# ZhangXiaze/DeepPointMap

Hardware: AMD Instinct MI355X
Metric: LiDAR frames/s (encode+match+register), 65 536 pts/frame (higher is better)
Workload: dtype f32 (attention scores K Q^T and P V, Linear / Conv1d (+ LayerNorm) layers with K <= 2048 as exact three-way bf16 splits: 6 bf16 products per fp32 product, fp32 accumulate -- fp32 accuracy, bf16 matrix pipe; all else fp32); 1 GPU; synthetic 64x65536-pt scans per GPU: Encoder.forward + consecutive-frame registration_forward (256x256) + information matrix per frame; points_per_frame=65536, parallelism=frame-sharded x1, one RCCL gather of descriptors+edges per step, weights=procedural (deeppointmap_amd/weights.py), allocator_reserve_gib=16, geometry_waits_for_caller_stream=True

## Files before the change

deeppointmap_amd/_lib.py:

```python
from __future__ import annotations

import ctypes
import os

import torch
from ctypes import c_char_p, c_double, c_int, c_longlong, c_size_t, c_uint, c_void_p

_HERE = os.path.dirname(os.path.abspath(__file__))
LIB_PATH = os.environ.get("DPM_LIB") or os.path.join(_HERE, "libdpm_hip.so")
VERSION_EXPERIMENT = 0x40000000

P, I, D, LL = c_void_p, c_int, c_double, c_longlong

SIGNATURES = {
    "dpm_version": (I, []),
    "dpm_error_string": (c_char_p, [I]),
    "dpm_prepare_points": (I, [P, P, I, I, I, P, P, P]),
    "dpm_to_channel_first": (I, [P, I, I, I, P, P]),
    "dpm_to_channel_first_ld": (I, [P, I, I, I, P, I, P]),
    "dpm_emit_descriptors": (I, [P, P, P, I, I, I, D, P, P, P, P, P]),
    "dpm_nested_levels": (I, [P, P, I, I, I, P, P, P, P, P]),
    "dpm_gather_frames": (I, [P, LL, I, I, I, P, I, P, P]),
    "dpm_fps_workspace_bytes": (c_size_t, [I, I, I]),
    "dpm_fps": (I, [P, P, I, I, I, P, P, P, P, P]),
    "dpm_fps_ex": (I, [P, P, I, I, I, P, P, P, P, I, P]),
    "dpm_fps_start": (I, [P, P, P, I, I, I, P, P, P, P, P]),
    "dpm_knn_workspace_bytes": (c_size_t, [I, I]),
    "dpm_knn_hybrid": (I, [P, P, P, I, I, I, I, D, P, P, P]),
    "dpm_knn_hybrid_reuse": (I, [P, P, P, I, I, I, I, D, P, P, P, P, P]),
    "dpm_knn_build_grid": (I, [P, P, I, I, D, P, P]),
    "dpm_knn_hybrid_prebuilt": (I, [P, P, P, I, I, I, I, D, P, P, P]),
    "dpm_ball_query": (I, [P, P, P, I, I, I, I, D, P, P]),
    "dpm_voxel_sampler_bounds": (I, [P, P, I, I, I, D, D, P, P]),
    "dpm_voxel_sampler_workspace_bytes": (c_size_t, [I, I, LL]),
    "dpm_voxel_sampler_select": (I, [P, P, I, I, I, D, D, P, LL, I, P, I, P, P, P]),
    "dpm_posegraph_optimize": (I, [P, I, P, P, P, P, I, I, P, P, P]),
    "dpm_host_topk_replay": (I, [P, I, I, I, P]),
    "dpm_host_sort_replay": (I, [P, I, I, P]),
    "dpm_group_mlp_max": (I, [P, P, P, P, P, P, P, P, I, I, I, I, I, I, D, P, P]),
    "dpm_group_mlp_max_generic": (I, [P, P, P, P, P, P, P, P, I, I, I, I, I, I, D, P, P]),
    "dpm_group_mlp_max_from_xyz": (I, [P, P, P, P, P, P, P, P, P, I, I, I, I, I, I, D, P, P]),
    "dpm_group_gather_ln_max": (I, [P, P, P, P, P, I, P, P, I, I, I, I, I, D, P, P]),
    "dpm_group_gather_ln_max_folded": (I, [P, P, P, P, I, P, P, I, I, I, I, I, D, P, P]),
    "dpm_group_affine_ln_max": (I, [P, P, P, P, P, P, I, P, P, I, I, I, I, I, D, P, P]),
    "dpm_group_gather_ln_max_centred": (I, [P, P, P, P, I, P, P, I, I, I, I, I, D, P, P]),
    "dpm_group_affine_ln_max_centred": (I, [P, P, P, P, P, P, I, P, P, I, I, I, I, I, D, P, P]),
    "dpm_linear": (I, [P, I, P, I, P, P, I, P, I, I, I, I, I, P]),
    "dpm_linear_batched": (I, [P, I, LL, P, I, LL, P, P, I, LL, P, I, LL, I, I, I, I, I, P]),
    "dpm_split_bf16x3": (I, [P, LL, P, P]),
    "dpm_linear_bf16x3": (I, [P, I, P, I, LL, P, P, I, P, I, I, I, I, I, P]),
    "dpm_linear_bf16x3_rank3": (I, [P, I, P, I, LL, P, P, I, P, I, I, I, I, I, P, P, I, D, P]),
    "dpm_linear_layernorm_bf16x3": (I, [P, I, P, I, LL, P, P, P, P, P, P, I, I, I, I, I, P]),
    "dpm_pwconv_pair_bf16x3": (I, [P, I, P, LL, P, P, P, P, LL, P, P, P, P, P, I, I, I, P]),
    "dpm_decoder_tail_bf16x3": (I, [P, P, P, P, I, I, P, LL, P, P, P, P, LL, P, P, LL, P, P, P, P]),
    "dpm_layernorm": (I, [P, I, P, P, P, P, P, I, I, I, I, P]),
    "dpm_linear_layernorm": (I, [P, I, P, I, P, P, P, P, P, P, I, I, I, I, I, P]),
    "dpm_three_interp_cat": (I, [P, P, P, P, P, I, I, I, I, I, P, P]),
    "dpm_posemb": (I, [P, I, P, I, I, I, P, P]),
    "dpm_attention": (I, [P, I, LL, P, I, LL, P, I, LL, P, I, LL, I, I, I, I, I, P]),
    "dpm_attention_shifted": (I, [P, I, LL, P, I, LL, P, I, LL, P, I, LL, I, I, I, I, I, I, P]),
    "dpm_attention_masked": (I, [P, I, LL, P, I, LL, P, I, LL, P, I, LL, I, I, I, I, I, I, P, P]),
    "dpm_attention_indexed": (I, [P, I, LL, P, I, LL, P, I, LL, P, I, LL, I, I, I, I, I, I, P, P]),
    "dpm_attention_split_workspace_bytes": (c_size_t, [I, I, I, I, I]),
    "dpm_attention_planes_bytes": (c_size_t, [I, I, I]),
    "dpm_attention_planes": (I, [P, I, LL, P, P, I, LL, I, I, I, I, I, P, P]),
    "dpm_linear_bf16x3_kvplanes": (I, [P, I, P, I, LL, P, P, I, I, I, I, I, I, I, P, P]),
    "dpm_attention_split": (I, [P, I, LL, P, I, LL, P, I, LL, P, I, LL, I, I, I, I, I, I, I, P, P]),
    "dpm_l2_normalize": (I, [P, I, I, P, P]),
    "dpm_match_workspace_bytes": (c_size_t, [I, I, I, I]),
    "dpm_match_topk": (I, [P, P, I, I, I, I, D, I, P, P, P, P]),
    "dpm_pairing_workspace_bytes": (c_size_t, [I, I, I]),
    "dpm_dual_softmax_topk": (I, [P, I, I, I, D, I, P, P, P, P]),
    "dpm_gather_pairs": (I, [P, P, P, I, I, I, I, I, P, P, P, P]),
    "dpm_mean_rows": (I, [P, I, I, I, P, I, P]),
    "dpm_kabsch_workspace_bytes": (c_size_t, [I, I]),
    "dpm_corr_kabsch": (I, [P, P, I, LL, P, I, LL, P, P, P, I, I, D, I, D, P, P, P, I, P]),
    "dpm_preprocess_workspace_bytes": (c_size_t, [LL]),
    "dpm_preprocess_scan": (I, [P, I, I, D, D, D, D, LL, P, P, I, P, P, P]),
    "dpm_knn_self_workspace_bytes": (c_size_t, [I]),
    "dpm_knn_self": (I, [P, I, I, D, P, P, P, P, P]),
    "dpm_point_normals": (I, [P, I, D, P, P, P]),
    "dpm_lowpass_similarity": (I, [P, P, I, I, I, P, P]),
    "dpm_stat_filter": (I, [P, I, D, I, D, P, P, P, P, P, P]),
    "dpm_filter_dc_workspace_bytes": (c_size_t, [I, I]),
    "dpm_outlier_filter_dc": (I, [P, P, P, I, I, D, D, D, P, P, P, P, P]),
    "dpm_lowpass_filter_dc": (I, [P, P, P, I, D, I, D, I, D, D, P, P, P, P, P]),
    "dpm_augment_workspace_bytes": (c_size_t, [I, LL]),
    "dpm_ground_filter": (I, [P, P, P, I, I, I, D, D, I, P, P, P, P, P]),
    "dpm_voxel_select": (I, [P, P, P, I, D, I, LL, P, P, P, P, P]),
    "dpm_mask_select": (I, [P, P, P, I, I, D, D, P, D, P, I, P, P, P, P, P]),
    "dpm_points_affine": (I, [P, P, I, I, P, P, P]),
    "dpm_points_deskew": (I, [P, P, P, I, I, P, I, I, P, D, P]),
    "dpm_gather_points": (I, [P, P, P, I, P, I, I, P, P, P, P]),
    "dpm_pack_frames": (I, [P, P, P, I, I, P, P, P, P]),
    "dpm_ingest_frames": (I, [P, P, LL, I, I, I, P, P, P, P, P]),
    "dpm_map_tile": (I, [P, P, P, P, I, I, I, P, P]),
    "dpm_infomat_workspace_bytes": (c_size_t, [I, I, I]),
    "dpm_information_matrix": (I, [P, I, P, I, P, D, P, P, P]),
    "dpm_information_matrix_batched": (I, [P, I, P, P, I, P, I, D, P, I, P, P]),
    "dpm_infomat_build_grids": (I, [P, I, P, I, D, P, P]),
    "dpm_infomat_search_grids": (I, [P, I, P, P, I, P, I, D, P, I, P, P]),
    "dpm_icp_workspace_bytes": (c_size_t, [I, I]),
    "dpm_icp_refine_batched": (I, [P, I, I, P, P, P, P, I, P, I, P, P, I, D, D, P, P, P, P, P, P, P, P, P]),
    "dpm_voxel_map_workspace_bytes": (c_size_t, [LL]),
    "dpm_voxel_map_init": (I, [LL, P, P]),
    "dpm_voxel_map_bounds": (I, [P, P, P, I, LL, P, P]),
# ... 121 lines not shown
```

deeppointmap_amd/csrc/gemm_b3.hip:

```cpp
#include "dpm_common.h"
#include <type_traits>

namespace {

using bf16x8 = __attribute__((ext_vector_type(8))) __bf16;
using f32x4 = __attribute__((ext_vector_type(4))) float;
using u32x4 = __attribute__((ext_vector_type(4))) unsigned;
using u32x2 = __attribute__((ext_vector_type(2))) unsigned;

__device__ __forceinline__ float b3_act(float v, int act) {
    if (act == DPM_ACT_RELU) return fmaxf(v, 0.f);
    if (act == DPM_ACT_SIGMOID) return 1.f / (1.f + __expf(-v));
    return v;
}

__global__ __launch_bounds__(256) void split_bf16x3_kernel(const float *__restrict__ W, long long n, uint16_t *__restrict__ planes) {
    const long long i = (long long)blockIdx.x * 256 + threadIdx.x;
    if (i >= n) return;
    unsigned h, m, l;
    split3(W[i], h, m, l);
    planes[i] = (uint16_t)(h >> 16), planes[n + i] = (uint16_t)(m >> 16), planes[2 * n + i] = (uint16_t)(l >> 16);
}

#ifndef DPM_B3_WIDE
// ... 689 lines not shown
        f32x4 y[2] = {f32x4{0.f, 0.f, 0.f, 0.f}, f32x4{0.f, 0.f, 0.f, 0.f}};
#pragma unroll
        for (int s4 = 0; s4 < PW_H / 32; ++s4) {
            unsigned hh[8], mm[8], ll[8];
#pragma unroll
            for (int e = 0; e < 8; ++e) split3(h[2 * s4 + (e >> 2)][e & 3], hh[e], mm[e], ll[e]);
            bf16x8 hb[3];
            hb[0] = __builtin_bit_cast(bf16x8, u32x4{pack2(hh[0], hh[1]), pack2(hh[2], hh[3]), pack2(hh[4], hh[5]), pack2(hh[6], hh[7])});
            hb[1] = __builtin_bit_cast(bf16x8, u32x4{pack2(mm[0], mm[1]), pack2(mm[2], mm[3]), pack2(mm[4], mm[5]), pack2(mm[6], mm[7])});
            hb[2] = __builtin_bit_cast(bf16x8, u32x4{pack2(ll[0], ll[1]), pack2(ll[2], ll[3]), pack2(ll[4], ll[5]), pack2(ll[6], ll[7])});
            bf16x8 a[2][3];
#pragma unroll
            for (int jj = 0; jj < 2; ++jj)
#pragma unroll
                for (int pl = 0; pl < 3; ++pl)
                    a[jj][pl] = *reinterpret_cast<const bf16x8 *>(&W2s[pl][s4][jj * 16 + fr][b3_col(fr, 8 * g)]);
#define DPM_PW2(PWQ, PXQ)                                                                             \
    _Pragma("unroll") for (int jj = 0; jj < 2; ++jj)                                                  \
        y[jj] = __builtin_amdgcn_mfma_f32_16x16x32_bf16(a[jj][PWQ], hb[PXQ], y[jj], 0, 0, 0)
            DPM_PW2(1, 1);
            DPM_PW2(2, 0);
            DPM_PW2(0, 2);
            DPM_PW2(1, 0);
            DPM_PW2(0, 1);
            DPM_PW2(0, 0);
#undef DPM_PW2
        }
        float s2 = 0.f;
#pragma unroll
        for (int jj = 0; jj < 2; ++jj) {
            const f32x4 bv = *reinterpret_cast<const f32x4 *>(&vec2[0][16 * jj + 4 * g]);
#pragma unroll
            for (int q = 0; q < 4; ++q) y[jj][q] += bv[q], s2 += y[jj][q];
        }
        const float mu2 = pw_rows4_sum(s2) * (1.f / PW_C);
        float q2 = 0.f;
#pragma unroll
        for (int jj = 0; jj < 2; ++jj)
#pragma unroll
            for (int q = 0; q < 4; ++q) y[jj][q] -= mu2, q2 = fmaf(y[jj][q], y[jj][q], q2);
        const float rs2 = rsqrtf(pw_rows4_sum(q2) * (1.f / PW_C) + 1e-5f);
        if (row0 + fr < R) {
#pragma unroll
            for (int jj = 0; jj < 2; ++jj) {
                const f32x4 gv = *reinterpret_cast<const f32x4 *>(&vec2[1][16 * jj + 4 * g]);
                const f32x4 ev = *reinterpret_cast<const f32x4 *>(&vec2[2][16 * jj + 4 * g]);
                const f32x4 pv = jj ? p1 : p0;
                f32x4 o;
#pragma unroll
                for (int q = 0; q < 4; ++q) o[q] = fmaxf(fmaf(y[jj][q] * rs2, gv[q], ev[q]) + pv[q], 0.f);
                *reinterpret_cast<f32x4 *>(out + (size_t)row * PW_C + 16 * jj + 4 * g) = o;
            }
        }
    }
}

}

extern "C" int dpm_split_bf16x3(const float *W, long long n, void *planes, dpm_stream_t stream) {
    DPM_CHECK_ARG(W && planes && n >= 1);
    hipLaunchKernelGGL(split_bf16x3_kernel, dim3(dpm_cdiv(n, 256)), dim3(256), 0, (hipStream_t)stream, W, n, (uint16_t *)planes);
    return dpm_launch_status();
}

extern "C" int dpm_linear_bf16x3_rank3(const float *x, int ldx, const void *w_planes, int ldw, long long plane_stride,
                                       const float *bias, const float *residual, int ldr, float *out, int ldo, int R, int Cin,
                                       int Cout, int act, const float *x3, const float *w3, int ldw3, double scale,
                                       dpm_stream_t stream);

extern "C" int dpm_linear_bf16x3(const float *x, int ldx, const void *w_planes, int ldw, long long plane_stride, const float *bias,
                                 const float *residual, int ldr, float *out, int ldo, int R, int Cin, int Cout, int act,
                                 dpm_stream_t stream) {
    return dpm_linear_bf16x3_rank3(x, ldx, w_planes, ldw, plane_stride, bias, residual, ldr, out, ldo, R, Cin, Cout, act, nullptr,
                                   nullptr, 0, 0.0, stream);
}

extern "C" int dpm_linear_bf16x3_rank3(const float *x, int ldx, const void *w_planes, int ldw, long long plane_stride,
                                       const float *bias, const float *residual, int ldr, float *out, int ldo, int R, int Cin,
                                       int Cout, int act, const float *x3, const float *w3, int ldw3, double scale,
                                       dpm_stream_t stream) {
    DPM_CHECK_ARG((x3 == nullptr) == (w3 == nullptr) && (!x3 || ldw3 >= 3));
    const float r3s = (float)scale;
    DPM_CHECK_ARG(x && w_planes && out && R >= 1 && Cin >= 1 && Cout >= 1 && ldx >= Cin && ldw >= Cin && ldo >= Cout);
    DPM_CHECK_ARG(act >= DPM_ACT_NONE && act <= DPM_ACT_SIGMOID && (!residual || ldr >= Cout) && plane_stride >= (long long)Cout * ldw);
    auto al = [](const void *p) { return ((uintptr_t)p & 15) == 0; };
    if (Cin % B3_KT != 0 || Cout % 4 != 0 || ldw % 8 != 0 || plane_stride % 8 != 0 || ldo % 4 != 0 || !al(w_planes) || !al(out) ||
        !al(bias) || (residual && (!al(residual) || ldr % 4 != 0)))
        return DPM_EUNSUPPORTED;
    const bool xvec = ldx % 4 == 0 && al(x);
    const long long big = (long long)dpm_cdiv(R, 64) * dpm_cdiv(Cout, 64);
#define DPM_B3_LAUNCH(TM, TN, V, PF)                                                                                          \
    hipLaunchKernelGGL((gemm_b3_kernel<TM, TN, V, PF>), dim3(dpm_cdiv(Cout, TN), dpm_cdiv(R, TM)), dim3(256), 0, (hipStream_t)stream, x, ldx, \
                       (const uint16_t *)w_planes, ldw, plane_stride, bias, residual, ldr, out, ldo, R, Cin, Cout, act, x3, w3, ldw3, r3s)
    if (DPM_B3_WIDE && xvec && Cout % 128 == 0 && (long long)dpm_cdiv(R, 64) * (Cout / 128) >= DPM_B3_WIDE) {
        DPM_B3_LAUNCH(64, 128, true, 1);
    } else if (big >= 192 || (R > 1024 && Cout > 32)) {
        const bool small = big <= DPM_B3_DEEP;
        if (xvec && small) DPM_B3_LAUNCH(64, 64, true, 4);
        else if (xvec) DPM_B3_LAUNCH(64, 64, true, 1);
        else if (small) DPM_B3_LAUNCH(64, 64, false, 4);
        else DPM_B3_LAUNCH(64, 64, false, 1);
    } else {
        const bool small = (long long)dpm_cdiv(R, 32) * dpm_cdiv(Cout, 32) <= 2 * DPM_B3_DEEP;
        if (xvec && small) DPM_B3_LAUNCH(32, 32, true, 4);
        else if (xvec) DPM_B3_LAUNCH(32, 32, true, 1);
        else if (small) DPM_B3_LAUNCH(32, 32, false, 4);
// ... 33 lines not shown
    auto al = [](const void *p) { return ((uintptr_t)p & 15) == 0; };
    if (Cin % B3_KT != 0 || ldx % 4 != 0 || ldw % 8 != 0 || plane_stride % 8 != 0 || ldo % 4 != 0 || !al(x) || !al(w_planes) ||
        !al(bias) || !al(pre) || !al(gamma) || !al(beta) || !al(post) || !al(out))
        return DPM_EUNSUPPORTED;
    hipStream_t st = (hipStream_t)stream;
#define DPM_GLN3(BM, BN, WGM, WGN)                                                                                             \
    hipLaunchKernelGGL((gemm_ln_b3_kernel<BM, BN, WGM, WGN>), dim3(dpm_cdiv(R, BM)), dim3(64 * WGM * WGN), 0, st, x, ldx,       \
                       (const uint16_t *)w_planes, ldw, plane_stride, bias, pre, gamma, beta, post, out, ldo, R, Cin, act)
    if (Cout == 256) DPM_GLN3(64, 256, 2, 4);
    else if (Cout == 128) DPM_GLN3(64, 128, 2, 2);
    else if (Cout == 64) DPM_GLN3(64, 64, 2, 2);
    else if (Cout == 32) DPM_GLN3(64, 32, 2, 2);
    else return DPM_EUNSUPPORTED;
#undef DPM_GLN3
    return dpm_launch_status();
}

#ifndef DPM_TAIL_ZREG
#define DPM_TAIL_ZREG 0
#endif
extern "C" int dpm_decoder_tail_bf16x3(const float *a, const float *pre, const float *post, float *out, int R, int C,
                                       const void *wo_planes, long long plane_o, const float *bo, const float *g2, const float *be2,
                                       const void *w0_planes, long long plane_0, const float *b0, const void *w2_planes,
                                       long long plane_2, const float *b2, const float *g3, const float *be3, dpm_stream_t stream) {
    DPM_CHECK_ARG(a && pre && out && wo_planes && w0_planes && w2_planes && g2 && be2 && g3 && be3 && R >= 1 && C >= 1 && a != out);
    const long long cc = (long long)C * C;
    DPM_CHECK_ARG(plane_o >= cc && plane_0 >= cc && plane_2 >= cc);
    auto al = [](const void *p) { return ((uintptr_t)p & 15) == 0; };
    if (C != DT_C || plane_o % 8 != 0 || plane_0 % 8 != 0 || plane_2 % 8 != 0 || !al(a) || !al(pre) || !al(post) || !al(out) ||
        !al(wo_planes) || !al(w0_planes) || !al(w2_planes) || !al(bo) || !al(b0) || !al(b2) || !al(g2) || !al(be2) || !al(g3) || !al(be3))
        return DPM_EUNSUPPORTED;
    const TailArgs A{a, pre, post, out, {(const uint16_t *)wo_planes, (const uint16_t *)w0_planes, (const uint16_t *)w2_planes},
                     {plane_o, plane_0, plane_2}, {bo, b0, b2}, g2, be2, g3, be3, R};
    hipLaunchKernelGGL(decoder_tail_b3_kernel<DPM_TAIL_ZREG != 0>, dim3(dpm_cdiv(R, DT_BM)), dim3(DT_T), 0, (hipStream_t)stream, A);
    return dpm_launch_status();
}

extern "C" int dpm_pwconv_pair_bf16x3(const float *x, int ldx, const void *w1_planes, long long plane1, const float *b1,
                                      const float *g1, const float *be1, const void *w2_planes_kperm, long long plane2,
                                      const float *b2, const float *g2, const float *be2, const float *post, float *out, int R,
                                      int C, int H, dpm_stream_t stream) {
    DPM_CHECK_ARG(x && w1_planes && w2_planes_kperm && g1 && be1 && g2 && be2 && out && R >= 1 && ldx >= C);
    auto al = [](const void *p) { return ((uintptr_t)p & 15) == 0; };
    if (C != PW_C || H != PW_H || ldx % 4 != 0 || plane1 % 8 != 0 || plane2 % 8 != 0 || !al(x) || !al(w1_planes) ||
        !al(w2_planes_kperm) || !al(post) || !al(out))
        return DPM_EUNSUPPORTED;
    const long long tiles = ((long long)R + 15) / 16;
    const int tpw = (int)std::max<long long>(1, (tiles + 4LL * DPM_PW_GRID - 1) / (4LL * DPM_PW_GRID));
    const unsigned grid = (unsigned)((tiles + 4LL * tpw - 1) / (4LL * tpw));
    hipLaunchKernelGGL(pwconv_pair_b3_kernel, dim3(grid), dim3(256), 0, (hipStream_t)stream, x, ldx, (const uint16_t *)w1_planes,
                       plane1, b1, g1, be1, (const uint16_t *)w2_planes_kperm, plane2, b2, g2, be2, post, out, R, tpw);
    return dpm_launch_status();
}
```

deeppointmap_amd/knobs.py:

```python
from __future__ import annotations

import os

FPS_ALGO = None
FUSED_LN = True
GEMM_BF16X3 = True
BF16X3_MAX_K = 2048
GEMM_LN_BF16X3 = True
BF16X3_LN_MIN_K = 128
FUSED_LN_SMALL_ROWS = 0
FOLD_GATHER = True
FOLD_MIN_RADIUS = 0.2
CENTRED_GATHER = True
FUSED_PWCONV = True
FUSED_MATCH = True
KV_PLANES = True
DECODER_TAIL_FUSED = True
DEDUP_FRAMES = True

_ENV = {"DPM_FOLD_MIN_RADIUS": ("FOLD_MIN_RADIUS", float), "DPM_KV_PLANES": ("KV_PLANES", lambda v: v != "0"), "DPM_CENTRED_GATHER": ("CENTRED_GATHER", lambda v: v != "0"), "DPM_FPS_ALGO": ("FPS_ALGO", int), "DPM_NO_FUSED_LN": ("FUSED_LN", lambda v: v != "1"),
        "DPM_DEDUP_FRAMES": ("DEDUP_FRAMES", lambda v: v != "0"), "DPM_DECODER_TAIL": ("DECODER_TAIL_FUSED", lambda v: v != "0"), "DPM_GEMM_BF16X3": ("GEMM_BF16X3", lambda v: v == "1"), "DPM_BF16X3_MAX_K": ("BF16X3_MAX_K", int), "DPM_BF16X3_LN_MIN_K": ("BF16X3_LN_MIN_K", int), "DPM_FUSED_LN_SMALL_ROWS": ("FUSED_LN_SMALL_ROWS", int), "DPM_GEMM_LN_BF16X3": ("GEMM_LN_BF16X3", lambda v: v == "1"),
        "DPM_FUSED_MATCH": ("FUSED_MATCH", lambda v: v != "0"), "DPM_FUSED_PWCONV": ("FUSED_PWCONV", lambda v: v != "0"), "DPM_FOLD_GATHER": ("FOLD_GATHER", lambda v: v != "0")}


def env_knobs() -> dict:
    return {k: v for k, v in sorted(os.environ.items()) if k.startswith("DPM_")}


def apply_env() -> dict:
    g = globals()
    for var, (name, conv) in _ENV.items():
        if var in os.environ:
            g[name] = conv(os.environ[var])
    return env_knobs()
```

deeppointmap_amd/ops.py:

```python
from __future__ import annotations

from typing import Optional, Tuple

import ctypes
import threading
import weakref

import torch

from . import _lib, knobs

ACT_NONE, ACT_RELU, ACT_SIGMOID = 0, 1, 2


def _ptr(t: Optional[torch.Tensor]):
    return None if t is None else t.data_ptr()


def _stream(t: torch.Tensor):
    return torch.cuda.current_stream(t.device).cuda_stream


def _chk(t: torch.Tensor, dtype, name: str):
    if not t.is_cuda:
# ... 470 lines not shown

def linear_layernorm(x: torch.Tensor, W: torch.Tensor, bias: Optional[torch.Tensor], gamma: torch.Tensor, beta: torch.Tensor,
                     act: int = ACT_NONE, pre: Optional[torch.Tensor] = None, post: Optional[torch.Tensor] = None) -> torch.Tensor:
    Cout, Cin = W.shape[0], W.shape[1]
    x2 = x.reshape(-1, x.shape[-1])
    if (knobs.GEMM_BF16X3 and knobs.GEMM_LN_BF16X3 and Cin % 32 == 0 and knobs.BF16X3_LN_MIN_K <= Cin <= knobs.BF16X3_MAX_K and Cout % 4 == 0 and W.numel() == Cout * Cin
            and x.dtype == torch.float32):
        wp = _weight_planes(W)
        if wp is not None and (bias is None or bias.data_ptr() % 16 == 0):
            if (Cout in FUSED_LN_WIDTHS and (x2.shape[0] >= FUSED_LN_MIN_ROWS or x2.shape[0] <= knobs.FUSED_LN_SMALL_ROWS)
                    and x2.is_contiguous() and knobs.FUSED_LN):
                planes, off, n = wp
                out = torch.empty(*x.shape[:-1], Cout, device=x.device, dtype=torch.float32)
                for nm, t in (("pre", pre), ("post", post)):
                    if t is not None:
                        _chk(t, torch.float32, nm)
                        if t.numel() != out.numel():
                            raise ValueError(f"{nm} must have the shape of the output")
                st = _lib.load().dpm_linear_layernorm_bf16x3(_ptr(x2), x2.stride(0), planes.data_ptr() + 2 * off, Cin, n, _ptr(bias),
                                                             _ptr(pre), _ptr(gamma), _ptr(beta), _ptr(post), _ptr(out), Cout,
                                                             x2.shape[0], Cin, Cout, act, _stream(x))
                if st == 0:
                    return out
                if st != -2:
                    _lib.check(st, "dpm_linear_layernorm_bf16x3")
            y = linear_bf16x3(x, W, bias, residual=pre)
            if y is not None:
                return layernorm(y, gamma, beta, act=act, post=post)
    if (Cout in FUSED_LN_WIDTHS and x2.shape[0] >= FUSED_LN_MIN_ROWS and W.is_contiguous() and x2.is_contiguous()
            and x.dtype == torch.float32 and Cin % 4 == 0 and knobs.FUSED_LN):
        _chk(W, torch.float32, "W")
        out = torch.empty(*x.shape[:-1], Cout, device=x.device, dtype=torch.float32)
        for n, t in (("pre", pre), ("post", post)):
            if t is not None:
                _chk(t, torch.float32, n)
                if t.numel() != out.numel():
                    raise ValueError(f"{n} must have the shape of the output")
        st = _lib.load().dpm_linear_layernorm(_ptr(x2), x2.stride(0), _ptr(W), Cin, _ptr(bias), _ptr(pre), _ptr(gamma),
                                              _ptr(beta), _ptr(post), _ptr(out), Cout, x2.shape[0], Cin, Cout, act, _stream(x))
        if st == 0:
            return out
        if st != -2:
            _lib.check(st, "dpm_linear_layernorm")
    y = linear(x, W, bias, residual=pre, exact=True)
    return layernorm(y, gamma, beta, act=act, post=post)


def _pwconv_kperm() -> torch.Tensor:
    return torch.tensor([16 * (2 * s + (e >> 2)) + 4 * g + (e & 3) for s in range(4) for g in range(4) for e in range(8)], dtype=torch.long)


def pwconv_pair(x: torch.Tensor, W1, b1, g1, be1, W2, b2, g2, be2, post: Optional[torch.Tensor]) -> Optional[torch.Tensor]:
    C, H = W1.shape[1], W1.shape[0]
    if not (knobs.FUSED_PWCONV and knobs.GEMM_BF16X3 and C == 32 and H == 128 and tuple(W2.shape[:2]) == (C, H) and x.is_cuda
            and x.dtype == torch.float32 and x.is_contiguous() and W1.numel() == C * H and W2.numel() == C * H):
        return None
    wp1 = _weight_planes(W1)
    if wp1 is None or (post is not None and (not post.is_contiguous() or post.numel() != x.numel())):
        return None
    for n, t_ in (("gamma1", g1), ("beta1", be1), ("gamma2", g2), ("beta2", be2)):
        _chk(t_, torch.float32, n)

    def make():
        Wp = W2.reshape(C, H)[:, _pwconv_kperm().to(W2.device)].contiguous()
        planes = torch.empty(3, C * H, device=W2.device, dtype=torch.int16)
        _lib.check(_lib.load().dpm_split_bf16x3(_ptr(Wp), C * H, _ptr(planes), _stream(W2)), "dpm_split_bf16x3")
        planes._dpm_keep = Wp
        return planes
    planes2 = _derived("bf16x3-planes-kperm", (W2,), make)
    planes1, off1, n1 = wp1
    x2 = x.reshape(-1, C)
    out = torch.empty_like(x)
    st = _lib.load().dpm_pwconv_pair_bf16x3(_ptr(x2), C, planes1.data_ptr() + 2 * off1, n1, _ptr(b1), _ptr(g1), _ptr(be1),
                                            planes2.data_ptr(), C * H, _ptr(b2), _ptr(g2), _ptr(be2), _ptr(post), _ptr(out),
                                            x2.shape[0], C, H, _stream(x))
    if st == -2:
        return None
    _lib.check(st, "dpm_pwconv_pair_bf16x3")
    return out


def decoder_tail(a: torch.Tensor, z1: torch.Tensor, Wo, bo, g2, be2, W0, b0, W2, b2, g3, be3,
                 post: Optional[torch.Tensor]) -> Optional[torch.Tensor]:
    C = a.shape[-1]
    if not (knobs.DECODER_TAIL_FUSED and knobs.GEMM_BF16X3 and knobs.GEMM_LN_BF16X3 and knobs.FUSED_LN and C == 256
            and knobs.BF16X3_LN_MIN_K <= C <= knobs.BF16X3_MAX_K and a.is_cuda and a.dtype == torch.float32 and a.dim() == 2
            and a.is_contiguous()):
        return None
    R = a.shape[0]
    if not (R >= FUSED_LN_MIN_ROWS or 1 <= R <= knobs.FUSED_LN_SMALL_ROWS):
        return None
    for t_ in (z1, post):
        if t_ is not None and not (t_.dtype == torch.float32 and t_.is_cuda and t_.is_contiguous() and tuple(t_.shape) == (R, C)):
            return None
    planes = []
    for W, b in ((Wo, bo), (W0, b0), (W2, b2)):
        if tuple(W.shape[:2]) != (C, C) or W.numel() != C * C or (b is not None and b.data_ptr() % 16):
            return None
        wp = _weight_planes(W)
        if wp is None:
            return None
        planes.append(wp)
    for n, t_ in (("gamma2", g2), ("beta2", be2), ("gamma3", g3), ("beta3", be3)):
        _chk(t_, torch.float32, n)
    out = torch.empty(R, C, device=a.device, dtype=torch.float32)
    (po, oo, no), (p0, o0, n0), (p2, o2, n2) = planes
    st = _lib.load().dpm_decoder_tail_bf16x3(_ptr(a), _ptr(z1), _ptr(post), _ptr(out), R, C, po.data_ptr() + 2 * oo, no, _ptr(bo),
                                             _ptr(g2), _ptr(be2), p0.data_ptr() + 2 * o0, n0, _ptr(b0), p2.data_ptr() + 2 * o2, n2,
                                             _ptr(b2), _ptr(g3), _ptr(be3), _stream(a))
    if st == -2:
        return None
    _lib.check(st, "dpm_decoder_tail_bf16x3")
    return out


def three_interp_cat(xyz1, xyz2, lengths2, fea1, fea2) -> torch.Tensor:
    for n, t in (("xyz1", xyz1), ("xyz2", xyz2), ("fea1", fea1), ("fea2", fea2)):
        _chk(t, torch.float32, n)
    _chk(lengths2, torch.int32, "lengths2")
    B, N, D1 = fea1.shape
    S, D2 = fea2.shape[1], fea2.shape[2]
    out = torch.empty(B, N, D1 + D2, device=fea1.device, dtype=torch.float32)
    _lib.check(_lib.load().dpm_three_interp_cat(_ptr(xyz1), _ptr(xyz2), _ptr(lengths2), _ptr(fea1), _ptr(fea2),
                                                B, N, S, D1, D2, _ptr(out), _stream(fea1)), "dpm_three_interp_cat")
    return out


def _rows2d(t: torch.Tensor, name: str) -> torch.Tensor:
    if t.dtype != torch.float32 or not t.is_cuda or t.dim() != 2 or t.stride(1) != 1:
        raise ValueError(f"{name}: expected a 2-D fp32 GPU tensor with unit column stride")
    return t
# ... 1913 lines not shown
```

include/dpm_hip.h:

```cpp
#ifndef DPM_HIP_H
#define DPM_HIP_H

#include <stddef.h>
#include <stdint.h>

#ifdef __cplusplus
extern "C" {
#endif

typedef void *dpm_stream_t;

#define DPM_OK 0
#define DPM_EINVAL (-1)
#define DPM_EUNSUPPORTED (-2)

#define DPM_ACT_NONE 0
#define DPM_ACT_RELU 1
#define DPM_ACT_SIGMOID 2

#define DPM_VERSION_EXPERIMENT 0x40000000
int dpm_version(void);
const char *dpm_error_string(int status);

int dpm_prepare_points(const float *points_cf, const uint8_t *padding, int B, int C, int N,
// ... 103 lines not shown


int dpm_posemb(const float *xyz, int ld, const float *dim_t, int F, int E, int R, float *out,
               dpm_stream_t stream);

int dpm_attention(const float *Q, int ldq, long long sq, const float *K, int ldk, long long sk,
                  const float *V, int ldv, long long sv, float *out, int ldo, long long so, int B, int M,
                  int N, int heads, int head_dim, dpm_stream_t stream);
int dpm_attention_shifted(const float *Q, int ldq, long long sq, const float *K, int ldk, long long sk,
                          const float *V, int ldv, long long sv, float *out, int ldo, long long so, int B, int M,
                          int N, int heads, int head_dim, int kv_shift, dpm_stream_t stream);

int dpm_attention_masked(const float *Q, int ldq, long long sq, const float *K, int ldk, long long sk,
                         const float *V, int ldv, long long sv, float *out, int ldo, long long so, int B, int M,
                         int N, int heads, int head_dim, int kv_shift, const uint8_t *key_mask, dpm_stream_t stream);

int dpm_attention_indexed(const float *Q, int ldq, long long sq, const float *K, int ldk, long long sk,
                          const float *V, int ldv, long long sv, float *out, int ldo, long long so, int B, int M,
                          int N, int heads, int head_dim, int kv_shift, const int32_t *seq_index, dpm_stream_t stream);

size_t dpm_attention_split_workspace_bytes(int B, int M, int heads, int head_dim, int nsplit);
int dpm_attention_split(const float *Q, int ldq, long long sq, const float *K, int ldk, long long sk, const float *V,
                        int ldv, long long sv, float *out, int ldo, long long so, int B, int M, int N, int heads,
                        int head_dim, int kv_shift, int nsplit, void *workspace, dpm_stream_t stream);

size_t dpm_attention_planes_bytes(int n_sequences, int N, int heads);
int dpm_linear_bf16x3_kvplanes(const float *x, int ldx, const void *w_planes, int ldw, long long plane_stride,
                               const float *bias, float *out, int ldo, int R, int Cin, int Cout, int kv_col0, int tokens,
                               int heads, void *kv_planes, dpm_stream_t stream);
int dpm_attention_planes(const float *Q, int ldq, long long sq, const void *kv_planes, float *out, int ldo, long long so,
                         int B, int M, int N, int heads, int kv_shift, const int32_t *seq_index, dpm_stream_t stream);

int dpm_split_bf16x3(const float *W, long long n, void *planes, dpm_stream_t stream);
int dpm_linear_bf16x3(const float *x, int ldx, const void *w_planes, int ldw, long long plane_stride, const float *bias,
                      const float *residual, int ldr, float *out, int ldo, int R, int Cin, int Cout, int act,
                      dpm_stream_t stream);
int dpm_linear_bf16x3_rank3(const float *x, int ldx, const void *w_planes, int ldw, long long plane_stride, const float *bias,
                            const float *residual, int ldr, float *out, int ldo, int R, int Cin, int Cout, int act,
                            const float *x3, const float *w3, int ldw3, double scale, dpm_stream_t stream);
int dpm_linear_layernorm_bf16x3(const float *x, int ldx, const void *w_planes, int ldw, long long plane_stride,
                                const float *bias, const float *pre, const float *gamma, const float *beta, const float *post,
                                float *out, int ldo, int R, int Cin, int Cout, int act, dpm_stream_t stream);

int dpm_decoder_tail_bf16x3(const float *a, const float *pre, const float *post, float *out, int R, int C, const void *wo_planes,
                            long long plane_stride_o, const float *bo, const float *gamma2, const float *beta2,
                            const void *w0_planes, long long plane_stride_0, const float *b0, const void *w2_planes,
                            long long plane_stride_2, const float *b2, const float *gamma3, const float *beta3,
                            dpm_stream_t stream);

int dpm_pwconv_pair_bf16x3(const float *x, int ldx, const void *w1_planes, long long plane_stride1, const float *b1,
                           const float *gamma1, const float *beta1, const void *w2_planes_kperm, long long plane_stride2,
                           const float *b2, const float *gamma2, const float *beta2, const float *post, float *out, int R,
                           int C, int H, dpm_stream_t stream);

int dpm_l2_normalize(const float *x, int R, int C, float *out, dpm_stream_t stream);

size_t dpm_match_workspace_bytes(int batch, int M, int N, int k);
int dpm_match_topk(const float *a, const float *b, int batch, int M, int N, int C, double tau, int k, float *out_val,
                   int32_t *out_idx, void *workspace, dpm_stream_t stream);

size_t dpm_pairing_workspace_bytes(int batch, int M, int N);
int dpm_dual_softmax_topk(float *S, int batch, int M, int N, double tau, int k, float *out_val,
                          int32_t *out_idx, void *workspace, dpm_stream_t stream);

int dpm_gather_pairs(const float *x, const float *y, const int32_t *flat_idx, int batch, int k, int M,
                     int N, int E, float *X, int32_t *src_idx, int32_t *dst_idx, dpm_stream_t stream);

int dpm_mean_rows(const float *x, int B, int R, int C, float *out, int ldo, dpm_stream_t stream);

size_t dpm_kabsch_workspace_bytes(int batch, int k);
int dpm_corr_kabsch(const float *offsets, const float *src_xyz, int ld_src, long long stride_src,
                    const float *dst_xyz, int ld_dst, long long stride_dst, const int32_t *src_idx,
                    const int32_t *dst_idx, const float *conf, int batch, int k, double eps_offset,
                    int num_iter, double std_ratio, void *workspace, float *result, float *header,
                    int header_stride, dpm_stream_t stream);


size_t dpm_preprocess_workspace_bytes(long long max_cells);
int dpm_preprocess_scan(const float *xyz, int N, int stride, double voxel_size, double min_dis, double max_dis,
                        double ratio, long long max_cells, float *out_xyz, int32_t *out_idx, int out_capacity,
                        int32_t *status, void *workspace, dpm_stream_t stream);

size_t dpm_knn_self_workspace_bytes(int N);
int dpm_knn_self(const float *xyz, int N, int K, double cell, int32_t *idx, float *dist2, float *mean_dist,
                 void *workspace, dpm_stream_t stream);
int dpm_point_normals(const float *xyz, int N, double radius, float *normals, void *workspace, dpm_stream_t stream);
int dpm_lowpass_similarity(const float *normals, const int32_t *idx, int N, int K, int flux, float *sim,
                           dpm_stream_t stream);
int dpm_stat_filter(const float *stat, int N, double k_std, int mode, double ratio, const float *xyz_in,
                    const int32_t *idx_in, float *xyz_out, int32_t *idx_out, int32_t *n_out, dpm_stream_t stream);

size_t dpm_filter_dc_workspace_bytes(int capacity, int K);
int dpm_outlier_filter_dc(const float *xyz, const int32_t *idx_in, const int32_t *count, int capacity, int nb_neighbors,
                          double std_ratio, double cell, double ratio, float *xyz_out, int32_t *idx_out,
                          int32_t *count_out, void *workspace, dpm_stream_t stream);
int dpm_lowpass_filter_dc(const float *xyz, const int32_t *idx_in, const int32_t *count, int capacity,
                          double normals_radius, int normals_num, double filter_std, int flux, double cell, double ratio,
                          float *xyz_out, int32_t *idx_out, int32_t *count_out, void *workspace, dpm_stream_t stream);


size_t dpm_augment_workspace_bytes(int capacity, long long cells);
int dpm_ground_filter(const float *xyz, const int32_t *idx_in, const int32_t *count, int capacity, int img_len,
                      int img_width, double grid_width, double ground_height, int preserve_sparse_ground, float *out_xyz,
                      int32_t *out_idx, int32_t *out_count, void *workspace, dpm_stream_t stream);
int dpm_voxel_select(const float *xyz, const int32_t *idx_in, const int32_t *count, int capacity, double voxel_size,
                     int retention, long long max_cells, float *out_xyz, int32_t *out_idx, int32_t *status,
// ... 274 lines not shown
```

Baseline: 16660 frames/s.

## Fuse 128->512->128 pointwise conv pair with LayerNorms into one bf16x3 kernel

Adds a fused HIP kernel for the wide (C=128, H=512) pointwise-conv pair. It runs the first GEMM, LayerNorm and ReLU with the hidden activations held in registers and LDS, then the second GEMM, LayerNorm, residual add and ReLU in the same kernel. Weight tiles are double-buffered through LDS. The aim is to remove the 64x512 fp32 hidden intermediate round-trip through global memory and the extra kernel launches. The cost is heavy LDS and register use per 512-thread block, which may limit occupancy.

```diff
diff --git a/deeppointmap_amd/_lib.py b/deeppointmap_amd/_lib.py
--- a/deeppointmap_amd/_lib.py
+++ b/deeppointmap_amd/_lib.py
@@ -52,6 +52,7 @@
     "dpm_linear_bf16x3_rank3": (I, [P, I, P, I, LL, P, P, I, P, I, I, I, I, I, P, P, I, D, P]),
     "dpm_linear_layernorm_bf16x3": (I, [P, I, P, I, LL, P, P, P, P, P, P, I, I, I, I, I, P]),
     "dpm_pwconv_pair_bf16x3": (I, [P, I, P, LL, P, P, P, P, LL, P, P, P, P, P, I, I, I, P]),
+    "dpm_pwconv_pair_wide_bf16x3": (I, [P, I, P, LL, P, P, P, P, LL, P, P, P, P, P, I, I, I, P]),
     "dpm_decoder_tail_bf16x3": (I, [P, P, P, P, I, I, P, LL, P, P, P, P, LL, P, P, LL, P, P, P, P]),
     "dpm_layernorm": (I, [P, I, P, P, P, P, P, I, I, I, I, P]),
     "dpm_linear_layernorm": (I, [P, I, P, I, P, P, P, P, P, P, I, I, I, I, I, P]),
diff --git a/deeppointmap_amd/csrc/gemm_b3.hip b/deeppointmap_amd/csrc/gemm_b3.hip
--- a/deeppointmap_amd/csrc/gemm_b3.hip
+++ b/deeppointmap_amd/csrc/gemm_b3.hip
@@ -765,6 +765,226 @@
                 *reinterpret_cast<f32x4 *>(out + (size_t)row * PW_C + 16 * jj + 4 * g) = o;
             }
         }
+    }
+}
+
+constexpr int PWW_C = 128, PWW_H = 512, PWW_BM = 64, PWW_T = 512, PWW_LDC = PWW_C + 4;
+constexpr int PWW_XT = 3 * PWW_BM * B3_LD, PWW_XP = PWW_BM * B3_LD;
+constexpr int PWW_WT = 3 * PWW_C * B3_LD, PWW_WP = PWW_C * B3_LD;
+constexpr int PWW_HK = 8;
+constexpr int PWW_N1 = (PWW_H / 128) * (PWW_C / B3_KT), PWW_N2 = PWW_H / B3_KT, PWW_NT = PWW_N1 + PWW_N2;
+struct PwwArgs {
+    const float *x;
+    int ldx;
+    const uint16_t *w1, *w2;
+    long long plane1, plane2;
+    const float *b1, *g1, *be1, *b2, *g2, *be2, *post;
+    float *out;
+    int R;
+};
+__global__ __launch_bounds__(PWW_T) void pwconv_wide_b3_kernel(PwwArgs A) {
+    __shared__ __attribute__((aligned(16))) uint16_t xh[PWW_HK * PWW_XT];
+    __shared__ __attribute__((aligned(16))) uint16_t wb[2][PWW_WT];
+    __shared__ float red[2][2][4][PWW_BM];
+    const int t = threadIdx.x, lane = t & 63, w = t >> 6, wm = w >> 2, wn = w & 3, fr = lane & 15, g = lane >> 4, fk = g * 8;
+    const int row0 = blockIdx.x * PWW_BM;
+    const int wrow = t >> 2, wk = (t & 3) * 8;
+    auto wsrc = [&](int it, int pl) {
+        it = min(it, PWW_NT - 1);
+        const uint16_t *p = it < PWW_N1 ? A.w1 + pl * A.plane1 + (size_t)((it >> 2) * 128 + wrow) * PWW_C + (it & 3) * B3_KT + wk
+                                        : A.w2 + pl * A.plane2 + (size_t)wrow * PWW_H + (it - PWW_N1) * B3_KT + wk;
+        return *reinterpret_cast<const u32x4 *>(p);
+    };
+    u32x4 wv[3];
+    auto wput = [&](int buf) {
+#pragma unroll
+        for (int pl = 0; pl < 3; ++pl) *reinterpret_cast<u32x4 *>(&wb[buf][pl * PWW_WP + wrow * B3_LD + b3_col(wrow, wk)]) = wv[pl];
+    };
+    auto put4 = [&](uint16_t *dst, const f32x4 &v) {
+        unsigned h0, m0, l0, h1, m1, l1, h2, m2, l2, h3, m3, l3;
+        split3(v[0], h0, m0, l0), split3(v[1], h1, m1, l1), split3(v[2], h2, m2, l2), split3(v[3], h3, m3, l3);
+        *reinterpret_cast<u32x2 *>(dst) = u32x2{pack2(h0, h1), pack2(h2, h3)};
+        *reinterpret_cast<u32x2 *>(dst + PWW_XP) = u32x2{pack2(m0, m1), pack2(m2, m3)};
+        *reinterpret_cast<u32x2 *>(dst + 2 * PWW_XP) = u32x2{pack2(l0, l1), pack2(l2, l3)};
+    };
+#pragma unroll
+    for (int pl = 0; pl < 3; ++pl) wv[pl] = wsrc(0, pl);
+    {
+        f32x4 xv[4];
+#pragma unroll
+        for (int p = 0; p < 4; ++p) {
+            const int e = p * PWW_T + t;
+            xv[p] = *reinterpret_cast<const f32x4 *>(A.x + (size_t)min(row0 + (e >> 5), A.R - 1) * A.ldx + (e & 31) * 4);
+        }
+        wput(0);
+#pragma unroll
+        for (int pl = 0; pl < 3; ++pl) wv[pl] = wsrc(1, pl);
+#pragma unroll
+        for (int p = 0; p < 4; ++p) {
+            const int e = p * PWW_T + t, r = e >> 5, k = (e & 31) * 4;
+            put4(&xh[(k >> 5) * PWW_XT + r * B3_LD + b3_col(r, k & 31)], xv[p]);
+        }
+    }
+    __syncthreads();
+    auto step = [&](int it, const uint16_t *xs, f32x4 (&acc)[2][2]) {
+        wput((it + 1) & 1);
+#pragma unroll
+        for (int pl = 0; pl < 3; ++pl) wv[pl] = wsrc(it + 2, pl);
+        const uint16_t *ws = wb[it & 1];
+        bf16x8 a[3][2], b[3][2];
+#pragma unroll
+        for (int pl = 0; pl < 3; ++pl) {
+#pragma unroll
+            for (int j = 0; j < 2; ++j) a[pl][j] = *reinterpret_cast<const bf16x8 *>(&ws[pl * PWW_WP + (wn * 32 + j * 16 + fr) * B3_LD + b3_col(fr, fk)]);
+#pragma unroll
+            for (int i = 0; i < 2; ++i) b[pl][i] = *reinterpret_cast<const bf16x8 *>(&xs[pl * PWW_XP + (wm * 32 + i * 16 + fr) * B3_LD + b3_col(fr, fk)]);
+        }
+#define DPM_B3(PWQ, PXQ)                                                                            \
+    _Pragma("unroll") for (int i = 0; i < 2; ++i) _Pragma("unroll") for (int j = 0; j < 2; ++j)     \
+        acc[i][j] = __builtin_amdgcn_mfma_f32_16x16x32_bf16(a[PWQ][j], b[PXQ][i], acc[i][j], 0, 0, 0)
+        DPM_B3(1, 1);
+        DPM_B3(2, 0);
+        DPM_B3(0, 2);
+        DPM_B3(1, 0);
+        DPM_B3(0, 1);
+        DPM_B3(0, 0);
+#undef DPM_B3
+        __syncthreads();
+    };
+    f32x4 h[4][2][2];
+#pragma unroll
+    for (int c = 0; c < 4; ++c)
+#pragma unroll
+        for (int i = 0; i < 2; ++i)
+#pragma unroll
+            for (int j = 0; j < 2; ++j) h[c][i][j] = f32x4{0.f, 0.f, 0.f, 0.f};
+#pragma unroll
+    for (int it = 0; it < PWW_N1; ++it) step(it, xh + (it & 3) * PWW_XT, h[it >> 2]);
+#pragma unroll
+    for (int c = 0; c < 4; ++c)
+#pragma unroll
+        for (int j = 0; j < 2; ++j) {
+            const f32x4 bv = A.b1 ? *reinterpret_cast<const f32x4 *>(A.b1 + c * 128 + wn * 32 + j * 16 + 4 * g) : f32x4{0.f, 0.f, 0.f, 0.f};
+#pragma unroll
+            for (int i = 0; i < 2; ++i) h[c][i][j] += bv;
+        }
+    auto lanes4 = [](float v) {
+        v += __shfl_xor(v, 16, 64);
+        return v + __shfl_xor(v, 32, 64);
+    };
+    auto waves4 = [&](int st, int i) {
+        const int r = wm * 32 + i * 16 + fr;
+        const float t0 = (red[st][0][0][r] + red[st][0][1][r]) + (red[st][0][2][r] + red[st][0][3][r]);
+        const float t1 = (red[st][1][0][r] + red[st][1][1][r]) + (red[st][1][2][r] + red[st][1][3][r]);
+        return t0 + t1;
+    };
+#pragma unroll
+    for (int i = 0; i < 2; ++i)
+#pragma unroll
+        for (int c = 0; c < 2; ++c) {
+            float e[2];
+#pragma unroll
+            for (int j = 0; j < 2; ++j) {
+                const f32x4 u = h[c][i][j], v = h[c + 2][i][j];
+                float s = 0.f;
+                s += (u[0] + u[1]) + (u[2] + u[3]);
+                s += (v[0] + v[1]) + (v[2] + v[3]);
+                e[j] = lanes4(s);
+            }
+            if (g == 0) red[0][c][wn][wm * 32 + i * 16 + fr] = e[0] + e[1];
+        }
+    __syncthreads();
+    float rs[2];
+#pragma unroll
+    for (int i = 0; i < 2; ++i) {
+        const float mu = waves4(0, i) / (float)PWW_H;
+#pragma unroll
+        for (int c = 0; c < 2; ++c) {
+            float e[2];
+#pragma unroll
+            for (int j = 0; j < 2; ++j) {
+                f32x4 &u = h[c][i][j], &v = h[c + 2][i][j];
+                u[0] -= mu, u[1] -= mu, u[2] -= mu, u[3] -= mu;
+                v[0] -= mu, v[1] -= mu, v[2] -= mu, v[3] -= mu;
+                float sq = 0.f;
+                sq = fmaf(u[0], u[0], fmaf(u[1], u[1], fmaf(u[2], u[2], fmaf(u[3], u[3], sq))));
+                sq = fmaf(v[0], v[0], fmaf(v[1], v[1], fmaf(v[2], v[2], fmaf(v[3], v[3], sq))));
+                e[j] = lanes4(sq);
+            }
+            if (g == 0) red[1][c][wn][wm * 32 + i * 16 + fr] = e[0] + e[1];
+        }
+    }
+    __syncthreads();
+#pragma unroll
+    for (int i = 0; i < 2; ++i) rs[i] = rsqrtf(waves4(1, i) / (float)PWW_H + 1e-5f);
+#pragma unroll
+    for (int c = 0; c < 4; ++c)
+#pragma unroll
+        for (int j = 0; j < 2; ++j) {
+            const int col = c * 128 + wn * 32 + j * 16 + 4 * g;
+            const f32x4 g4 = *reinterpret_cast<const f32x4 *>(A.g1 + col), b4 = *reinterpret_cast<const f32x4 *>(A.be1 + col);
+#pragma unroll
+            for (int i = 0; i < 2; ++i)
+#pragma unroll
+                for (int q = 0; q < 4; ++q) h[c][i][j][q] = fmaxf(fmaf(h[c][i][j][q] * rs[i], g4[q], b4[q]), 0.f);
+        }
+    auto put_half = [&](int c0) {
+#pragma unroll
+        for (int cc = 0; cc < 2; ++cc)
+#pragma unroll
+            for (int i = 0; i < 2; ++i)
+#pragma unroll
+                for (int j = 0; j < 2; ++j) {
+                    const int r = wm * 32 + i * 16 + fr;
+                    put4(&xh[(4 * cc + wn) * PWW_XT + r * B3_LD + b3_col(r, 16 * j + 4 * g)], h[c0 + cc][i][j]);
+                }
+    };
+    f32x4 y[2][2];
+#pragma unroll
+    for (int i = 0; i < 2; ++i)
+#pragma unroll
+        for (int j = 0; j < 2; ++j) y[i][j] = f32x4{0.f, 0.f, 0.f, 0.f};
+    put_half(0);
+    __syncthreads();
+#pragma unroll 2
+    for (int kt = 0; kt < PWW_HK; ++kt) step(PWW_N1 + kt, xh + kt * PWW_XT, y);
+    put_half(2);
+    __syncthreads();
+#pragma unroll 2
+    for (int kt = 0; kt < PWW_HK; ++kt) step(PWW_N1 + PWW_HK + kt, xh + kt * PWW_XT, y);
+    float *ct = reinterpret_cast<float *>(xh);
+#pragma unroll
+    for (int i = 0; i < 2; ++i)
+#pragma unroll
+        for (int j = 0; j < 2; ++j)
+            *reinterpret_cast<float4 *>(&ct[(wm * 32 + i * 16 + fr) * PWW_LDC + wn * 32 + j * 16 + g * 4]) =
+                make_float4(y[i][j][0], y[i][j][1], y[i][j][2], y[i][j][3]);
+    __syncthreads();
+    constexpr int G = PWW_C / 4, RPS = PWW_T / G;
+    const int cr = t / G, cc = (t % G) * 4;
+    const float4 bv = A.b2 ? *reinterpret_cast<const float4 *>(A.b2 + cc) : make_float4(0.f, 0.f, 0.f, 0.f);
+    const float4 g4 = *reinterpret_cast<const float4 *>(A.g2 + cc), b4 = *reinterpret_cast<const float4 *>(A.be2 + cc);
+    auto gsum = [](float v) {
+#pragma unroll
+        for (int off = 1; off < G; off <<= 1) v += __shfl_xor(v, off, 64);
+        return v;
+    };
+#pragma unroll
+    for (int p = 0; p < PWW_BM / RPS; ++p) {
+        const int r = row0 + p * RPS + cr, rr = min(r, A.R - 1);
+        float4 v = *reinterpret_cast<const float4 *>(&ct[(p * RPS + cr) * PWW_LDC + cc]);
+        v.x += bv.x, v.y += bv.y, v.z += bv.z, v.w += bv.w;
+        const float mu = gsum((v.x + v.y) + (v.z + v.w)) / (float)PWW_C;
+        v.x -= mu, v.y -= mu, v.z -= mu, v.w -= mu;
+        const float rs2 = rsqrtf(gsum(fmaf(v.x, v.x, fmaf(v.y, v.y, fmaf(v.z, v.z, v.w * v.w)))) / (float)PWW_C + 1e-5f);
+        float4 o = make_float4(fmaf(v.x * rs2, g4.x, b4.x), fmaf(v.y * rs2, g4.y, b4.y), fmaf(v.z * rs2, g4.z, b4.z),
+                               fmaf(v.w * rs2, g4.w, b4.w));
+        if (A.post) {
+            const float4 pv = *reinterpret_cast<const float4 *>(A.post + (size_t)rr * PWW_C + cc);
+            o.x += pv.x, o.y += pv.y, o.z += pv.z, o.w += pv.w;
+        }
+        o.x = fmaxf(o.x, 0.f), o.y = fmaxf(o.y, 0.f), o.z = fmaxf(o.z, 0.f), o.w = fmaxf(o.w, 0.f);
+        if (r < A.R) *reinterpret_cast<float4 *>(A.out + (size_t)r * PWW_C + cc) = o;
     }
 }
 
@@ -904,3 +1124,18 @@
                        plane1, b1, g1, be1, (const uint16_t *)w2_planes_kperm, plane2, b2, g2, be2, post, out, R, tpw);
     return dpm_launch_status();
 }
+
+extern "C" int dpm_pwconv_pair_wide_bf16x3(const float *x, int ldx, const void *w1_planes, long long plane1, const float *b1,
+                                           const float *g1, const float *be1, const void *w2_planes, long long plane2,
+                                           const float *b2, const float *g2, const float *be2, const float *post, float *out, int R,
+                                           int C, int H, dpm_stream_t stream) {
+    DPM_CHECK_ARG(x && w1_planes && w2_planes && g1 && be1 && g2 && be2 && out && R >= 1 && C >= 1 && H >= 1 && ldx >= C && x != out);
+    DPM_CHECK_ARG(plane1 >= (long long)C * H && plane2 >= (long long)C * H);
+    auto al = [](const void *p) { return ((uintptr_t)p & 15) == 0; };
+    if (C != PWW_C || H != PWW_H || ldx % 4 != 0 || plane1 % 8 != 0 || plane2 % 8 != 0 || !al(x) || !al(w1_planes) || !al(w2_planes) ||
+        !al(b1) || !al(g1) || !al(be1) || !al(b2) || !al(g2) || !al(be2) || !al(post) || !al(out))
+        return DPM_EUNSUPPORTED;
+    const PwwArgs A{x, ldx, (const uint16_t *)w1_planes, (const uint16_t *)w2_planes, plane1, plane2, b1, g1, be1, b2, g2, be2, post, out, R};
+    hipLaunchKernelGGL(pwconv_wide_b3_kernel, dim3(dpm_cdiv(R, PWW_BM)), dim3(PWW_T), 0, (hipStream_t)stream, A);
+    return dpm_launch_status();
+}
diff --git a/deeppointmap_amd/knobs.py b/deeppointmap_amd/knobs.py
--- a/deeppointmap_amd/knobs.py
+++ b/deeppointmap_amd/knobs.py
@@ -13,6 +13,7 @@
 FOLD_MIN_RADIUS = 0.2
 CENTRED_GATHER = True
 FUSED_PWCONV = True
+FUSED_PWCONV_WIDE = True
 FUSED_MATCH = True
 KV_PLANES = True
 DECODER_TAIL_FUSED = True
@@ -20,7 +21,7 @@
 
 _ENV = {"DPM_FOLD_MIN_RADIUS": ("FOLD_MIN_RADIUS", float), "DPM_KV_PLANES": ("KV_PLANES", lambda v: v != "0"), "DPM_CENTRED_GATHER": ("CENTRED_GATHER", lambda v: v != "0"), "DPM_FPS_ALGO": ("FPS_ALGO", int), "DPM_NO_FUSED_LN": ("FUSED_LN", lambda v: v != "1"),
         "DPM_DEDUP_FRAMES": ("DEDUP_FRAMES", lambda v: v != "0"), "DPM_DECODER_TAIL": ("DECODER_TAIL_FUSED", lambda v: v != "0"), "DPM_GEMM_BF16X3": ("GEMM_BF16X3", lambda v: v == "1"), "DPM_BF16X3_MAX_K": ("BF16X3_MAX_K", int), "DPM_BF16X3_LN_MIN_K": ("BF16X3_LN_MIN_K", int), "DPM_FUSED_LN_SMALL_ROWS": ("FUSED_LN_SMALL_ROWS", int), "DPM_GEMM_LN_BF16X3": ("GEMM_LN_BF16X3", lambda v: v == "1"),
-        "DPM_FUSED_MATCH": ("FUSED_MATCH", lambda v: v != "0"), "DPM_FUSED_PWCONV": ("FUSED_PWCONV", lambda v: v != "0"), "DPM_FOLD_GATHER": ("FOLD_GATHER", lambda v: v != "0")}
+        "DPM_FUSED_MATCH": ("FUSED_MATCH", lambda v: v != "0"), "DPM_FUSED_PWCONV": ("FUSED_PWCONV", lambda v: v != "0"), "DPM_FUSED_PWCONV_WIDE": ("FUSED_PWCONV_WIDE", lambda v: v != "0"), "DPM_FOLD_GATHER": ("FOLD_GATHER", lambda v: v != "0")}
 
 
 def env_knobs() -> dict:
diff --git a/deeppointmap_amd/ops.py b/deeppointmap_amd/ops.py
--- a/deeppointmap_amd/ops.py
+++ b/deeppointmap_amd/ops.py
@@ -546,6 +546,8 @@
 
 def pwconv_pair(x: torch.Tensor, W1, b1, g1, be1, W2, b2, g2, be2, post: Optional[torch.Tensor]) -> Optional[torch.Tensor]:
     C, H = W1.shape[1], W1.shape[0]
+    if (C, H) == (128, 512):
+        return _pwconv_pair_wide(x, W1, b1, g1, be1, W2, b2, g2, be2, post)
     if not (knobs.FUSED_PWCONV and knobs.GEMM_BF16X3 and C == 32 and H == 128 and tuple(W2.shape[:2]) == (C, H) and x.is_cuda
             and x.dtype == torch.float32 and x.is_contiguous() and W1.numel() == C * H and W2.numel() == C * H):
         return None
@@ -571,6 +573,35 @@
     if st == -2:
         return None
     _lib.check(st, "dpm_pwconv_pair_bf16x3")
+    return out
+
+
+def _pwconv_pair_wide(x, W1, b1, g1, be1, W2, b2, g2, be2, post) -> Optional[torch.Tensor]:
+    C, H = 128, 512
+    if not (knobs.FUSED_PWCONV_WIDE and knobs.GEMM_BF16X3 and knobs.GEMM_LN_BF16X3 and knobs.FUSED_LN and knobs.BF16X3_LN_MIN_K <= C
+            and H <= knobs.BF16X3_MAX_K and tuple(W2.shape[:2]) == (C, H) and W1.numel() == C * H and W2.numel() == C * H
+            and x.is_cuda and x.dtype == torch.float32 and x.shape[-1] == C and x.is_contiguous()):
+        return None
+    R = x.numel() // C
+    if not (R >= FUSED_LN_MIN_ROWS or 1 <= R <= knobs.FUSED_LN_SMALL_ROWS):
+        return None
+    if post is not None and not (post.dtype == torch.float32 and post.is_cuda and post.is_contiguous() and post.numel() == x.numel()):
+        return None
+    if any(b is not None and b.data_ptr() % 16 for b in (b1, b2)):
+        return None
+    wp1, wp2 = _weight_planes(W1), _weight_planes(W2)
+    if wp1 is None or wp2 is None:
+        return None
+    for n, t_ in (("gamma1", g1), ("beta1", be1), ("gamma2", g2), ("beta2", be2)):
+        _chk(t_, torch.float32, n)
+    (p1, o1, n1), (p2, o2, n2) = wp1, wp2
+    out = torch.empty_like(x)
+    st = _lib.load().dpm_pwconv_pair_wide_bf16x3(_ptr(x), C, p1.data_ptr() + 2 * o1, n1, _ptr(b1), _ptr(g1), _ptr(be1),
+                                                 p2.data_ptr() + 2 * o2, n2, _ptr(b2), _ptr(g2), _ptr(be2), _ptr(post), _ptr(out),
+                                                 R, C, H, _stream(x))
+    if st == -2:
+        return None
+    _lib.check(st, "dpm_pwconv_pair_wide_bf16x3")
     return out
 
 
diff --git a/include/dpm_hip.h b/include/dpm_hip.h
--- a/include/dpm_hip.h
+++ b/include/dpm_hip.h
@@ -179,6 +179,11 @@
                            const float *gamma1, const float *beta1, const void *w2_planes_kperm, long long plane_stride2,
                            const float *b2, const float *gamma2, const float *beta2, const float *post, float *out, int R,
                            int C, int H, dpm_stream_t stream);
+
+int dpm_pwconv_pair_wide_bf16x3(const float *x, int ldx, const void *w1_planes, long long plane_stride1, const float *b1,
+                                const float *gamma1, const float *beta1, const void *w2_planes, long long plane_stride2,
+                                const float *b2, const float *gamma2, const float *beta2, const float *post, float *out, int R,
+                                int C, int H, dpm_stream_t stream);
 
 int dpm_l2_normalize(const float *x, int R, int C, float *out, dpm_stream_t stream);
 
```

Result: no change. 16820 frames/s, median of 6 (+1.0%).
